# s10m/GPU-Tiled-QR-Decomposition

Hardware: AMD Instinct MI355X
Metric: fp64 QR GFLOP/s and %MFMA-peak, dense m×n, at 1/2/4/8 MI355X (higher is better)
Workload: dtype f64; 1 GPU; tiled QR 16384x16384 f64 storage, tile 256 (BASELINE configs[2]); m=16384, n=16384, tile=256, parallelism=single GPU, inputs=one resident copy per timed step, staged before the timed region, chain_segment_length=8

## Files before the change

gpu-tiled-qr-decomposition_amd/csrc/chain_asm.hpp:

```cpp
#pragma once
#ifdef TQR_C64_INC
#include TQR_C64_INC
#else
#include "chain_asm_gen.inc"
#endif

namespace tqr {

__device__ __forceinline__ __amdgpu_buffer_rsrc_t null_rsrc(const void* p) {
  const unsigned long long u = (unsigned long long)p;
  const unsigned lo = __builtin_amdgcn_readfirstlane((unsigned)u);
  const unsigned hi = __builtin_amdgcn_readfirstlane((unsigned)(u >> 32));
  return __builtin_amdgcn_make_buffer_rsrc((void*)(((unsigned long long)hi << 32) | lo), 0, 0, 0x00020000);
}

template <int B>
__device__ __forceinline__ void ca_load_strip_head(__amdgpu_buffer_rsrc_t xin, __amdgpu_buffer_rsrc_t hrs, unsigned loff) {
  if constexpr (B == 256)
    asm volatile("s_nop 4\n\t" TQR_CHAIN_ASM_STRIP_LOAD_B256 "\n\t" TQR_CHAIN_ASM_HEAD_LOAD
                 :: [loff] "v"(loff), [xin] "s"(xin), [hrs] "s"(hrs) : "memory", TQR_CHAIN_ASM_CLOBBERS);
  else
    asm volatile("s_nop 4\n\t" TQR_CHAIN_ASM_STRIP_LOAD_B128 "\n\t" TQR_CHAIN_ASM_HEAD_LOAD
                 :: [loff] "v"(loff), [xin] "s"(xin), [hrs] "s"(hrs) : "memory", TQR_CHAIN_ASM_CLOBBERS);
}

__device__ __forceinline__ unsigned sreg(unsigned v) {
  unsigned r;
  asm volatile("s_nop 1\n\tv_readfirstlane_b32 %0, %1" : "=s"(r) : "v"(v));
  return r;
}

#if TQR_CHAIN_ASM_COAL
#define TQR_CA_COAL_INS , [bpa] "v"(o.bpa), [loffc] "v"(o.loffc), [hoff] "s"(o.hoff)
#define TQR_CA_COAL_CLOB "vcc",
#else
#define TQR_CA_COAL_INS
#define TQR_CA_COAL_CLOB
#endif
struct CaGroup {
  unsigned vz, vx, vt, vl16, loff;
  const double* svsrc;
  const double* stsrc;
  unsigned sdst;
  int sw;
  __amdgpu_buffer_rsrc_t hrs;
  int goff, hsc;
  __amdgpu_buffer_rsrc_t xout, xin, hnx;
  unsigned bpa = 0, loffc = 0;
  int hoff = 0;
};
__device__ __forceinline__ unsigned coal_bpa(int lane) { return 4u * (unsigned)(((lane & 3) << 4) | (lane >> 3)); }
__device__ __forceinline__ unsigned coal_off(int lane, size_t ldm) {
  return (unsigned)(((size_t)(lane >> 3) * ldm + 2 * (lane & 7)) * sizeof(double));
}

template <int B, int KIND, int G = 0>
__device__ __forceinline__ void ca_group(const CaGroup& o) {
  unsigned m0s, st;
#define TQR_CA_INS                                                                                     \
  [vz] "v"(o.vz), [vx] "v"(o.vx), [vt] "v"(o.vt), [vl16] "v"(o.vl16), [loff] "v"(o.loff), [svsrc] "s"(o.svsrc), \
      [stsrc] "s"(o.stsrc), [sdst] "s"(o.sdst), [sw] "s"(o.sw), [hrs] "s"(o.hrs),                            \
      [goff] "s"(o.goff), [hsc] "s"(o.hsc), [xout] "s"(o.xout), [xin] "s"(o.xin),       \
      [hnx] "s"(o.hnx) TQR_CA_COAL_INS
#define TQR_CA_STMT(TEXT) \
  asm volatile(TEXT : [m0s] "=&s"(m0s), [st] "=&s"(st) : TQR_CA_INS : "memory", "scc", TQR_CA_COAL_CLOB TQR_CHAIN_ASM_CLOBBERS)
  if constexpr (KIND == 4) {
    static_assert(G >= 1 && G + 1 < B / 32, "UNMQR body: groups 1 .. NG-2");
    if constexpr (B == 256) {
      if constexpr (G == 1) TQR_CA_STMT(TQR_CHAIN_ASM_U1_B256);
      else if constexpr (G == 2) TQR_CA_STMT(TQR_CHAIN_ASM_U2_B256);
      else if constexpr (G == 3) TQR_CA_STMT(TQR_CHAIN_ASM_U3_B256);
      else if constexpr (G == 4) TQR_CA_STMT(TQR_CHAIN_ASM_U4_B256);
      else if constexpr (G == 5) TQR_CA_STMT(TQR_CHAIN_ASM_U5_B256);
      else TQR_CA_STMT(TQR_CHAIN_ASM_U6_B256);
    } else {
      if constexpr (G == 1) TQR_CA_STMT(TQR_CHAIN_ASM_U1_B128);
      else TQR_CA_STMT(TQR_CHAIN_ASM_U2_B128);
    }
  } else if constexpr (KIND == 5 || KIND == 6) {
    if constexpr (B == 256) {
      if constexpr (KIND == 5) TQR_CA_STMT(TQR_CHAIN_ASM_UHANDOVER_B256);
      else TQR_CA_STMT(TQR_CHAIN_ASM_UHANDOVERL_B256);
    } else {
      if constexpr (KIND == 5) TQR_CA_STMT(TQR_CHAIN_ASM_UHANDOVER_B128);
      else TQR_CA_STMT(TQR_CHAIN_ASM_UHANDOVERL_B128);
    }
  } else if constexpr (B == 256) {
    if constexpr (KIND == 0) TQR_CA_STMT(TQR_CHAIN_ASM_PLAIN_B256);
    else if constexpr (KIND == 1) TQR_CA_STMT(TQR_CHAIN_ASM_HANDOVER_B256);
    else if constexpr (KIND == 2) TQR_CA_STMT(TQR_CHAIN_ASM_HANDOVERL_B256);
    else TQR_CA_STMT(TQR_CHAIN_ASM_XIN_B256);
  } else {
    if constexpr (KIND == 0) TQR_CA_STMT(TQR_CHAIN_ASM_PLAIN_B128);
    else if constexpr (KIND == 1) TQR_CA_STMT(TQR_CHAIN_ASM_HANDOVER_B128);
    else if constexpr (KIND == 2) TQR_CA_STMT(TQR_CHAIN_ASM_HANDOVERL_B128);
    else TQR_CA_STMT(TQR_CHAIN_ASM_XIN_B128);
  }
#undef TQR_CA_STMT
#undef TQR_CA_INS
}

template <int B>
__device__ __forceinline__ void ca_ugroup(int g, const CaGroup& o) {
  if constexpr (B == 256) {
    switch (g) {
      case 1: ca_group<B, 4, 1>(o); break;
      case 2: ca_group<B, 4, 2>(o); break;
      case 3: ca_group<B, 4, 3>(o); break;
      case 4: ca_group<B, 4, 4>(o); break;
      case 5: ca_group<B, 4, 5>(o); break;
      default: ca_group<B, 4, 6>(o); break;
    }
  } else {
    if (g == 1) ca_group<B, 4, 1>(o);
// ... 155 lines not shown
  int* const tcs = sflag + 58;
  int* const fls = sflag + 59;
  int* const acs = sflag + 60;
  if (pw) {
    pv.reset();
    *lds_int(tcs) = -1;
    *lds_int(fls) = -1;
  }
  const bool remote = a.dist && tile_owner(k, a.world, a.cyclic) != a.rank;
  int* const rf = uni(a.Rf + (size_t)k * P * NG);
  const int ep = uni(a.epoch);
  int fl_pf = -1;
  auto ready = [&](int i_, int g_) -> bool {
    if (!remote) return pv.ensure(rc, g_, i_ - k + 1, err);
    const int fi = i_ * NG + g_;
    if (fi == fl_pf && lds_u(fls) >= ep) return true;
    return spin_ge_u(rf + fi, ep, err, true);
  };
  const unsigned lds0 = __builtin_amdgcn_readfirstlane((unsigned)(size_t)(const __attribute__((address_space(3))) void*)lds);
  const unsigned oz = (unsigned)((x * VP + y * NRI) * 8), ox = (unsigned)((y * VP + x * NRI) * 8);
  const unsigned ot = (unsigned)(G::VIMG * 8 + (x * 4 + y) * NRI * 8);
  const unsigned loff = head_off_pair<B>(ldm, 0);
  const unsigned vl16 = 16u * lane;
#if TQR_CHAIN_ASM_COAL
  const unsigned bpa = coal_bpa(lane), loffc = coal_off(lane, ldm);
  const int hoff = uni((int)(8 * ldm * sizeof(double)));
#endif
  FST(6);
  if (k == 0 && a.Uc) {
    const bool ok = pw ? spin_ge_u(&a.Uc[j], a.nxc, err) : true;
    if (!ca_sync<0, 5>(ok, pw, sflag, par)) return;
  }
  const int ifirst = seg == 0 ? k : i0;
  bool xin = false;
  bool xu = false;
  for (int i = ifirst; i < i1 || i == k; i = (i == k ? i0 : i + 1)) {
    const bool ts = i != k;
    S* const Xt = ts ? Aj + (size_t)i * B : At;
    const __amdgpu_buffer_rsrc_t hrs = head_rsrc(At + colo, ts);
    if (!xin) {
      bool ok = true;
      if (pw) {
        if (i == ifirst && seg > 0) ok = spin_ge_u(&acg[0], seg, err);
        FST(9);
        if (ok && k > 0) ok = spin_ge_u(tc(i), k, err);
        FST(8);
        if (ok) ok = ready(i, 0);
      }
      FST(j == k + 1 ? 18 : 19);
      CA_MARK(5);
      if (!ca_sync<0, 5>(ok, pw, sflag, par)) return;
      CA_RESTART();
#ifdef TQR_FLOW_STAMPS
      if (t == 0 && i == ifirst) {
        const int idx = sflag[-1];
        if (idx < (1 << 18)) g_ttl[3 * idx + 2] += (__builtin_amdgcn_s_memrealtime() - g_ttl[3 * idx]) << 16;
      }
#endif
      FST(7);
      ca_dma<B>(vimg(i, 0), timg(i, 0), sreg(lds0 + (unsigned)(buf * BUF * 8)), w, vl16);
      ca_load_strip_head<B>(uniform_rsrc(Xt + colo), hrs, loff);
      FST(4);
    }
    const int inext = uni((i == k) ? i0 : i + 1);
    const bool has_next = uni(inext < i1 ? 1 : 0) != 0;
    bool okall = true;
    for (int g = 0; g < NG && okall; ++g) {
      bool ok = true;
      CA_MARK(7);
      const bool pp = pw;
      if (pp) {
        if (g + 1 == NG && has_next && k > 0 && lds_u(tcs) < k) ok = spin_ge_u(tc(inext), k, err);
        if (ok && i == ifirst && seg > 0 && g + 1 < NG && !(g > 0 && lds_u(acs) >= seg))
          ok = spin_ge_u(&acg[g + 1], seg, err);
        if (ok) {
          if (g + 1 < NG) ok = ready(i, g + 1);
          else if (has_next) ok = ready(inext, 0);
        }
      }
      FST(j == k + 1 ? 20 : 0);
      CA_MARK(2);
      constexpr int NHO = 2 * NP + 8 < 63 ? 2 * NP + 8 : 63;
      constexpr int XL = B == 256 ? TQR_CHAIN_ASM_XLEAD_B256 : TQR_CHAIN_ASM_XLEAD_B128;
      constexpr int NHL = NP + XL + 8 < 63 ? NP + XL + 8 : 63;
// ... 20 lines not shown
        const int tg = next_test_group<NG>(g);
        const bool here = g + 2 < NG;
        if (here || has_next) {
          if (!remote) {
            if (pfw) lds_prefetch_u(rc + tg, pv.rv + tg, false);
          } else if (pw) {
            fl_pf = (here ? i : inext) * NG + tg;
            lds_prefetch_u(rf + fl_pf, fls, true);
          }
        }
        if (pw && g + 2 == NG && has_next && k > 0) lds_prefetch_u(tc(inext), tcs, false);
        if (pw && i == ifirst && seg > 0 && g + 2 < NG) lds_prefetch_u(&acg[g + 2], acs, false);
      }
      FST(7);
      CA_RESTART();
      const int gd = g + 1 < NG ? g + 1 : has_next ? 0 : g, id = g + 1 < NG ? i : has_next ? inext : i;
      const unsigned vb = lds0 + (unsigned)(buf * BUF * 8);
      CaGroup o;
      o.vz = vb + oz;
      o.vx = vb + ox;
      o.vt = vb + ot;
      o.vl16 = vl16;
      o.loff = loff;
      o.svsrc = vimg(id, gd);
      o.stsrc = timg(id, gd);
      o.sdst = sreg(lds0 + (unsigned)((buf ^ 1) * BUF * 8));
      o.sw = w;
      o.hrs = hrs;
      o.hsc = (int)sreg(has_next ? 0u : 1u);
      o.goff = uni(g * IB * 8);
#if TQR_CHAIN_ASM_COAL
      o.bpa = bpa;
      o.loffc = loffc;
      o.hoff = hoff;
#endif
      CA_MARK(3);
      const bool ue = !ts && uskip;
      if (g + 1 < NG) {
        if (ue && g > 0) {
          o.xout = uniform_rsrc(Xt + colo);
          ca_ugroup<B>(g, o);
        } else if (g == 0 && xin && late) {
          o.xin = uniform_rsrc(Xt + colo);
          ca_group<B, 3>(o);
        } else {
          ca_group<B, 0>(o);
// ... 38 lines not shown
```

gpu-tiled-qr-decomposition_amd/csrc/flow_list.hpp:

```cpp
#pragma once

#if defined(__HIPCC__)
#define TQR_HD __host__ __device__
#else
#define TQR_HD
#endif

namespace tqr {

struct Item {
  int ts, l, m, k;
};

inline bool valid_b(int b) { return b == 16 || b == 32 || b == 64 || b == 128 || b == 256; }

constexpr int T_CHAIN = 4;
constexpr int T_UP = 5, T_DOWN = 6;

template <int NW_, int IB_, int WPC_>
struct FlowShape {
  static constexpr int NW = NW_, NT = 64 * NW_, SW = 16 * NW_, IB = IB_, WPC = WPC_;
};
using ShapeW8 = FlowShape<8, 32, 1>;
using ShapeW4 = FlowShape<4, 16, 2>;
// ... 6 lines not shown

TQR_HD inline int tile_owner(int j, int world, int cyclic = 0) {
  const int blk = j / world, r = j - blk * world;
  if (cyclic) return r;
  return (blk & 1) ? world - 1 - r : r;
}

TQR_HD inline int seglen_of_chain(int k, int j, int kmax, int seglen, int seglen_la, int la_tail,
                                  int tail = 0, int tail_sl = 1) {
  if (k >= kmax - tail) return tail_sl;
  if (j != k + 1) return seglen;
  return k >= kmax - la_tail ? 1 : seglen_la;
}
TQR_HD inline bool unmqr_alone(int k, int j, int kmax, int ualone) { return j == k + 1 && k >= kmax - ualone; }
TQR_HD inline int nseg_of_chain(int k, int j, int p, int kmax, int sl, int ualone) {
  const int rows = p - k - 1;
  if (rows <= 0) return 1;
  return (rows + sl - 1) / sl + (unmqr_alone(k, j, kmax, ualone) ? 1 : 0);
}
TQR_HD inline int seg_of_row(int k, int j, int i, int kmax, int sl, int ualone) {
  return (i - k - 1) / sl + (unmqr_alone(k, j, kmax, ualone) ? 1 : 0);
}

}
```

gpu-tiled-qr-decomposition_amd/csrc/flowplan.cpp:

```cpp
#include "flowplan.hpp"

#include <cstdlib>
#include <cstring>
#include <functional>
#include <map>
#include <queue>
#include <string>
#include <tuple>
#include <unordered_map>

#include "gridscheduler.h"

namespace tqr {

int flow_shape(int dtype, int b) {
  if (dtype != TQR_F64) return 8;
  const char* e = getenv("TQR_FLOW_SHAPE");
  if (e && strcmp(e, "w4") == 0) return 4;
  if (e && strcmp(e, "r") == 0 && b == 256) return 5;
  return 8;
}

namespace {
using u64 = unsigned long long;
// ... 534 lines not shown
int tqr_flow_plan_check(int M, int N, int b, int seglen, int* ntasks, int* est_order) {
  return list_check(spec64(M, N, b, seglen), ntasks, est_order);
}

int tqr_flow_xfer_plan_check(int M, int N, int b, int seglen, int nxc, double tcol, int* ntasks, int* est_order) {
  if (nxc < 1) return TQR_EINVAL;
  return list_check(spec64(M, N, b, seglen, 1, -1, nxc, tcol), ntasks, est_order);
}

int tqr_dist_plan_check(int M, int N, int b, int seglen, int rank, int world, int* ntasks, int* nfwd) {
  if (rank < 0 || seglen < 1) return TQR_EINVAL;
  FlowPlan fp;
  if (flow_list(spec64(M, N, b, seglen, world, rank), fp) != TQR_OK) return TQR_EINVAL;
  if (ntasks) *ntasks = (int)fp.items.size();
  if (nfwd) {
    int c = 0;
    if (world > 1)
      for (auto& it : fp.items) c += (it.ts & 0xff) != T_CHAIN;
    *nfwd = c;
  }
  return TQR_OK;
}

int tqr_flow_strip_width(void) { return shape_info(flow_shape(TQR_F64, 256)).sw; }

int tqr_flow_order_check(int M, int N, int b, const int* items, int n) {
  if (M <= 0 || N <= 0 || !valid_b(b) || !items || n <= 0) return TQR_EINVAL;
  std::vector<Item> L(n);
  for (int x = 0; x < n; ++x) L[x] = Item{items[4 * x], items[4 * x + 1], items[4 * x + 2], items[4 * x + 3]};
  return flow_list_topological(L, M, N, shape_ns(flow_shape(TQR_F64, b), b)) ? 1 : 0;
}

}
```

gpu-tiled-qr-decomposition_amd/csrc/plans.hip:

```cpp
#include <hip/hip_runtime.h>

#include <algorithm>
#include <cstdio>
#include <cstdlib>
#include <cstring>
#include <mutex>
#include <new>
#include <tuple>
#include <vector>

#include "gridscheduler.h"
#include "plan.hpp"
#include "solve.hpp"
#include "tqr.h"
#include "wave_dev.hpp"

using namespace tqr;

tqr::PlanShape tqr::plan_shape(const tqr_plan* pl) { return PlanShape{pl->m, pl->n, pl->b, pl->dtype, pl->kmax, pl->capped}; }

extern "C" {

const char* tqr_strerror(int s) {
  switch (s) {
// ... 117 lines not shown
  pl->ldsU = lds_update(b);
  if (hipEventCreate(&pl->ev0) != hipSuccess || hipEventCreate(&pl->ev1) != hipSuccess ||
      hipEventCreateWithFlags(&pl->evDone, hipEventDisableTiming) != hipSuccess) {
    tqr_plan_destroy(pl); return TQR_EHIP;
  }
  pl->shape = flow_shape(dtype, b);
  pl->nt = shape_info(pl->shape).nt;
  pl->ns = shape_ns(pl->shape, b);
  pl->ng = b / shape_ib(pl->shape, b);
  if (pl->engine == TQR_ENGINE_FLOW) {
    int dev = 0;
    hipDeviceProp_t pr;
    if (hipGetDevice(&dev) != hipSuccess || hipGetDeviceProperties(&pr, dev) != hipSuccess) {
      tqr_plan_destroy(pl); return TQR_EHIP;
    }
    const int full_grid = pr.multiProcessorCount * shape_info(pl->shape).wpc;
    pl->grid = full_grid;
    if (const char* gs = getenv("TQR_FLOW_GRID")) pl->grid = std::max(1, atoi(gs));
    FlowPlan fp;
    pl->knobs = flow_knobs(pl->p, pl->q, dtype, world, pl->grid >= full_grid, 0, steps, b);
    if (const char* eca = getenv("TQR_CHAIN_ASM")) pl->chain_asm = atoi(eca) & 3;
    if (const char* eu = getenv("TQR_UNMQR_SKIP"); eu && atoi(eu) == 0 && pl->chain_asm) pl->chain_asm |= 4;
    if (const char* e32 = getenv("TQR_CHAIN32_ASM"); e32 && atoi(e32) == 0) pl->chain_asm |= 8;
    build_flow_plan(pl->p, pl->q, pl->ns, pl->ng, pl->knobs, fp, nullptr, steps);
    pl->nflow_global = (int)fp.items.size();
    pl->list_hash = flow_list_hash(fp.items);
    if (world > 1) partition_flow_plan(fp, rank, world);
    pl->nflow = (int)fp.items.size();
    pl->est_order = fp.est_order;
    pl->sync_ints = 4 + 3 * (size_t)pl->kmax * pl->ng + (size_t)pl->p * pl->q * pl->ns +
                    (size_t)pl->kmax * pl->q * pl->ns * pl->ng + (size_t)pl->q;
    if (pl->nflow <= 0 || hipMalloc(&pl->d_flow, sizeof(Item) * pl->nflow) != hipSuccess ||
        hipMalloc(&pl->d_sync, sizeof(int) * pl->sync_ints) != hipSuccess ||
        hipMalloc(&pl->d_wk, sizeof(double*) * pl->kmax) != hipSuccess) {
      tqr_plan_destroy(pl); return TQR_ENOMEM;
    }
    const bool wk_uc = world > 1 && !(getenv("TQR_DIST_WK_CACHED") && atoi(getenv("TQR_DIST_WK_CACHED")) == 1);
    for (int k = 0; k < pl->kmax; ++k) {
      double* w = nullptr;
      const size_t wb = wk_bytes(b, pl->p - k, dtype, shape_ib(pl->shape, b));
      if ((wk_uc ? hipExtMallocWithFlags((void**)&w, wb, hipDeviceMallocUncached) : hipMalloc(&w, wb)) != hipSuccess) {
        tqr_plan_destroy(pl); return TQR_ENOMEM;
      }
      pl->wk.push_back(w);
    }
    if (hipMemcpy(pl->d_wk, pl->wk.data(), sizeof(double*) * pl->kmax, hipMemcpyHostToDevice) != hipSuccess) {
// ... 103 lines not shown
```

gpu-tiled-qr-decomposition_amd/gen/gen_chain_asm.py:

```python
#!/usr/bin/env python3
import os
import sys

NW = 8
IB = 32
NRI = IB // 4
VP = IB + 2
VPB = VP * 8

sys.path.insert(0, os.path.dirname(os.path.abspath(__file__)))
import gfx950_hazards as HZ

W_MF_C, W_MF_AB, W_MF_VALU, W_MF_ST = HZ.F64["srcc"], HZ.F64["srcab"], HZ.F64["valu"], HZ.F64["vmem"]
W_VALU_MF, W_VALU_ST, W_ST_WAR, W_M0 = HZ.VALU_TO_MFMA, HZ.VALU_TO_STORE, HZ.STORE_WAR, HZ.M0_TO_LDS_DMA

OP0, Z0, WR0, H0, X0 = 32, 80, 96, 112, 128
HP0 = 128
VTMP1, VDMA, VTMP2 = 96, 97, 80
VLO = 32


AG = 512


# ... 121 lines not shown

    def wait_lgkm(self, tags):
        idx = [self.lgkm.index(t) for t in tags if t in self.lgkm]
        if not idx:
            return
        k = len(self.lgkm) - 1 - max(idx)
        assert k <= 15
        self.emit(f"s_waitcnt lgkmcnt({k})")
        self.lgkm = self.lgkm[len(self.lgkm) - k:] if k else []

    def text(self):
        return "\\n\\t".join(self.lines)


class Body:

    def __init__(self, B, handover, nw=NW, xbank=None, resident=False, after_switch=False, xlead=None, xin_from=None,
                 skip=0, early_st=(), early_ld=()):
        self.B, self.NKS, self.NP = B, B // 4, B // 8
        self.handover = handover
        self.nw = nw
        self.X0 = X0 if xbank is None else AG + 128 * xbank
        self.coal = COAL and nw == 8 and xbank is None
        self.s = Stream()
        vimg = (B * VP + 127) // 128 * 128
        self.VIMG = vimg
        self.NIV, self.NIT = vimg // 128, (16 * NRI * NRI + 127) // 128
        self.PV, self.PT = -(-self.NIV // nw), -(-self.NIT // nw)
        self.STEPS = self.PV + self.PT
        self.s.vm = [f"X{p}" for p in range(self.NP)] + ["H"]
        self.xlead, self.xin_from = xlead, xin_from
        if xin_from is not None:
            self.s.vm = [f"X{p}" for p in range(xin_from)] + ["H"]
        self.skip, self.early_st, self.early_ld = skip, list(early_st), list(early_ld)
        assert skip % 8 == 0 and 0 <= skip < self.NKS and (xin_from is None or not skip)
        self.resident = resident
        if resident:
            assert not handover and xbank is not None and nw == 4
            self.s.vm = [f"X{p}" for p in RES_LD_SCHED[-1]] if after_switch else []

    def p1_slot(self, ks):
        return OP0 + 16 * (ks % 3)

    def t_slot(self, kb):
        return OP0 + 16 * (1 + kb % 2)

# ... 60 lines not shown

        K0 = self.skip
        dma_at = {}
        for m in range(self.STEPS):
            dma_at.setdefault(K0 + int((m + 0.5) * (NKS - K0) / self.STEPS), []).append(m)
        vtmp_set = False

        def need_vtmp(ks):
            nonlocal vtmp_set
            if ks < NKS and ks * 4 * VPB + 48 >= 65536 and not vtmp_set:
                s.emit(f"v_add_u32 v{VTMP1}, 0x8000, %[vz]")
                vtmp_set = True

        early = [("st", p) for p in self.early_st] + [("ld", p) for p in self.early_ld]
        for ks in range(K0, min(K0 + D, NKS)):
            need_vtmp(ks)
            p1_reads(ks)
        for ks in range(K0, NKS):
            nxt = ks + D
            need_vtmp(nxt)
            if self.xin_from is not None and ks % 2 == 0:
                for p in range(self.xin_from, self.NP):
                    if max(0, 2 * (p - self.xin_from)) == ks:
                        s.vmem_load(self.X0 + 4 * p, f"buffer_load_dwordx4 {vq(self.X0 + 4 * p)}, %[loff], %[xin], 0 "
                                    f"offen offset:{64 * p} sc1 nt", f"XI{p}")
            if ks % 2 == 0:
                s.wait_vm(f"X{ks // 2}")
            s.wait_lgkm([f"z{ks}.{h}" for h in range(4)])
            sl = self.p1_slot(ks)
            for r in range(NRI):
                s.mfma(Z0 + 2 * r, sl + 2 * r, self.X0 + 2 * ks, "0" if ks == K0 else Z0 + 2 * r)
                if nxt < NKS and r in (1, 3, 5, 7):
                    h = (r - 1) // 2
                    off = nxt * 4 * VPB + 16 * h
                    base, o = self.lds("%[vz]", off, VTMP1)
                    s.ds_read(self.p1_slot(nxt) + 4 * h, base, o, f"z{nxt}.{h}")
                if r == 2:
                    for m in dma_at.get(ks, []):
                        self.dma_step(m)
                if r == 5 and early:
                    for _ in range(-(-len(early) // (NKS - ks))):
                        self.strip_io(*early.pop(0))
        assert not early
        def t_reads(kb):
            for h in range(4):
                s.ds_read(self.t_slot(kb) + 4 * h, "%[vt]", kb * 1024 + 16 * h, f"t{kb}.{h}")

        units = [(b, half, pp) for b in range(K0 // 4, NKS // 4) for half in range(2) for pp in range(2)]
# ... 143 lines not shown
            self.s.emit("s_waitcnt lgkmcnt(0)")

    CT = (H0, H0 + 8)

    def coal_bperm(self, q):
        s = self.s
        for h in range(2):
            t = self.CT[h]
            for d in range(4):
                s.ds_bperm(t + d, self.X0 + 4 * (2 * q) + d, 32 * h, f"bp{q}.{h}.a{d}")
                s.ds_bperm(t + 4 + d, self.X0 + 4 * (2 * q + 1) + d, 32 * h, f"bp{q}.{h}.b{d}")

    def coal_store(self, q):
        s = self.s
        for h in range(2):
            t = self.CT[h]
            s.wait_lgkm([f"bp{q}.{h}.{ab}{d}" for ab in "ab" for d in range(4)])
            for d in range(4):
                s.valu_cnd(t + d, t + d, t + 4 + d)
            so = "%[hoff]" if h else "0"
            s.vmem_store(t, f"buffer_store_dwordx4 {vq(t)}, %[loffc], %[xout], {so} offen offset:{128 * q} sc1",
                         f"XS{2 * q + h}")

    def strip_io(self, kind, p):
        s = self.s
        r = self.X0 + 4 * p
        if kind == "st":
            s.vmem_store(r, f"buffer_store_dwordx4 {vq(r)}, %[loff], %[xout], 0 offen offset:{64 * p} sc1", f"XS{p}")
        else:
            s.vmem_load(r, f"buffer_load_dwordx4 {vq(r)}, %[loff], %[xin], 0 offen offset:{64 * p} sc1 nt", f"XL{p}")


def simulate(B, bodies, nelem=3, seglen_last=True, ubodies=None):
    NG, NP = B // IB, B // 8
    plain, ho = bodies[0], bodies[1]
    xin = bodies[2] if len(bodies) > 2 else None
    lead = ho.xlead if ho.xlead is not None else NP
    out = []
    stored, loaded = {}, {}

    def wait(k):
        while len(out) > k:
            out.pop(0)

    def done(pred, what):
        bad = [o for o in out if pred(o)]
        assert not bad, f"B={B}: {what}: {bad[:3]} still outstanding"

    def play(body, e, g):
        for ev in body.s.events:
            if ev[0] == "vm":
                tag = ev[1]
                if tag.startswith("D"):
# ... 47 lines not shown
            else:
                play(ho if g + 1 == NG else xin if (xin is not None and g == 0 and e > 0) else plain, e, g)
    wait(0)
    for e in range(nelem):
        assert sorted(stored.get(e, [])) == list(range(NP)), f"B={B}: strip stores of element {e}"
        if e > 0:
            assert sorted(loaded.get(e, [])) == list(range(NP)), f"B={B}: strip loads of element {e}"
    return True


def dma_job(B, nw=NW):
    body = Body(B, False, nw)
    st = body.s
    st.emit("s_nop 4")
    st.emit("s_mov_b32 %[m0s], m0")
    for m in range(body.STEPS):
        body.dma_step(m)
    st.emit("s_mov_b32 m0, %[m0s]")
    return st.text()


def strip_load(B, x0=X0):
    NP = B // 8
    lines = [f"buffer_load_dwordx4 {vq(x0 + 4 * p)}, %[loff], %[xin], 0 offen offset:{64 * p} sc1 nt" for p in range(NP)]
    return "\\n\\t".join(lines)


def head_load():
    lines = [f"buffer_load_dwordx4 {vq(H0 + 4 * h)}, %[loff], %[hrs], 0 offen offset:{64 * h} sc1" for h in range(4)]
    return "\\n\\t".join(lines)


def strip_store(B, x0=X0):
    NP = B // 8
    lines = [f"buffer_store_dwordx4 {vq(x0 + 4 * p)}, %[loff], %[xout], 0 offen offset:{64 * p} sc1" for p in range(NP)]
    lines.append("s_nop 1")
    return "\\n\\t".join(lines)


STAMPS = bool(os.environ.get("GEN_STAMPS"))
COAL = bool(os.environ.get("GEN_COALESCE"))
XLEAD = int(os.environ.get("GEN_XLEAD", "2"))
NOPRIO = bool(os.environ.get("GEN_NOPRIO"))
PWPRIO = bool(os.environ.get("GEN_PWPRIO"))
PRIOREV = bool(os.environ.get("GEN_PRIOREV"))

RES_ST_SCHED = [list(range(0, 16)), list(range(16, 32))]
RES_LD_SCHED = [list(range(0, 6)), list(range(6, 12)), list(range(12, 17)), list(range(17, 22)),
                list(range(22, 27)), list(range(27, 32))]


def _lines(ls):
    return "\\n\\t".join(ls)


def res_xst(g, bank):
    x0 = 128 * bank
    ls = ["s_nop 4"]
    ls += [f"buffer_store_dwordx4 a[{x0 + 4 * p}:{x0 + 4 * p + 3}], %[loff], %[xout], 0 offen offset:{64 * p} sc1"
           for p in RES_ST_SCHED[g]]
    return _lines(ls)

# ... 6 lines not shown
    return _lines(ls)


def res_head(g, store):
    ls = ["s_nop 4"]
    for h in range(4):
        r = HP0 + 16 * g + 4 * h
        op = "buffer_store_dwordx4" if store else "buffer_load_dwordx4"
        ls.append(f"{op} v[{r}:{r + 3}], %[loff], %[hrs], 0 offen offset:{256 * g + 64 * h} sc1")
    if store:
        ls.append("s_nop 1")
    return _lines(ls)


def res_park_zero():
    return _lines([f"v_mov_b64 v[{r}:{r + 1}], 0" for r in range(HP0, 256, 2)])


def res_park_from(bank):
    return _lines(["s_nop 7"] + [f"v_accvgpr_read_b32 v{HP0 + i}, a{128 * bank + i}" for i in range(128)] + ["s_nop 1"])


def main():
    out = sys.argv[1] if len(sys.argv) > 1 else "csrc/chain_asm_gen.inc"
    parts = ["// GENERATED by gen/gen_chain_asm.py -- do not edit. fp64 chain group bodies (gfx950).", "#pragma once"]
    stats = []
    for B in (128, 256):
        built = {}
        for ho in (False, True):
            body = Body(B, ho)
            s = body.build()
            built[ho] = body
            name = f"TQR_CHAIN_ASM_{'HANDOVER' if ho else 'PLAIN'}_B{B}"
            parts.append(f'#define {name} "{s.text()}"')
            nm = sum(1 for l in s.lines if l.startswith("v_mfma"))
            nn = sum(int(l.split()[1]) + 1 for l in s.lines if l.startswith("s_nop"))
            stats.append(f"// {name}: {len(s.lines)} lines, {nm} MFMAs, {nn} nop states, {s.clock} issue slots")
        for n in (1, 2, 3, 5):
            simulate(B, (built[False], built[True]), nelem=n)
        lead = XLEAD
        hol = Body(B, True, xlead=lead)
        hol.build()
        xb = Body(B, False, xin_from=lead)
        xb.build()
        for n in (1, 2, 3, 5):
            simulate(B, (built[False], hol, xb), nelem=n)
        for nm, bd in ((f"TQR_CHAIN_ASM_HANDOVERL_B{B}", hol), (f"TQR_CHAIN_ASM_XIN_B{B}", xb)):
            parts.append(f'#define {nm} "{bd.s.text()}"')
            nmf = sum(1 for l in bd.s.lines if l.startswith("v_mfma"))
            stats.append(f"// {nm}: {len(bd.s.lines)} lines, {nmf} MFMAs, {bd.s.clock} issue slots")
        NG = B // IB
        for late in (False, True):
            ub = {}
            for g in range(1, NG):
                lo = 4 * g
                if g + 1 < NG:
                    ub[g] = Body(B, False, skip=8 * g, early_st=range(4 * (g - 1), lo))
                else:
                    ub[g] = Body(B, True, xlead=lead if late else None, skip=8 * g, early_st=range(4 * (g - 1), lo),
                                 early_ld=[p for p in range(lo) if not late or p < lead])
                ub[g].build()
            for n in (1, 2, 3, 5):
                if late:
                    simulate(B, (built[False], hol, xb), nelem=n, ubodies=ub)
                else:
                    simulate(B, (built[False], built[True]), nelem=n, ubodies=ub)
            names = [(f"TQR_CHAIN_ASM_UHANDOVER{'L' if late else ''}_B{B}", ub[NG - 1])]
            parts.append(f"#define TQR_CHAIN_ASM_UHANDOVER{'L' if late else ''}_SYNC_B{B} {ub[NG - 1].sync_after()}")
            if not late:
                names += [(f"TQR_CHAIN_ASM_U{g}_B{B}", ub[g]) for g in range(1, NG - 1)]
            for nm, bd in names:
                parts.append(f'#define {nm} "{bd.s.text()}"')
                nmf = sum(1 for l in bd.s.lines if l.startswith("v_mfma"))
                stats.append(f"// {nm}: {len(bd.s.lines)} lines, {nmf} MFMAs, {bd.s.clock} issue slots")
        parts.append(f"#define TQR_CHAIN_ASM_XLEAD_B{B} {lead}")
        if B == 128:
            parts.append(f"#define TQR_CHAIN_ASM_COAL {1 if COAL else 0}")
        parts.append(f'#define TQR_CHAIN_ASM_DMA_B{B} "{dma_job(B)}"')
        parts.append(f'#define TQR_CHAIN_ASM_STRIP_LOAD_B{B} "{strip_load(B)}"')
        parts.append(f'#define TQR_CHAIN_ASM_STRIP_STORE_B{B} "{strip_store(B)}"')
    parts.append(f'#define TQR_CHAIN_ASM_HEAD_LOAD "{head_load()}"')
    regs = ", ".join(f'"v{i}"' for i in range(VLO, 256))
    parts.append(f"#define TQR_CHAIN_ASM_CLOBBERS {regs}")
    B = 256
    built = {}
    for ho in (False, True):
        body = Body(B, ho, nw=4, xbank=0)
        s = body.build()
        built[ho] = body
        name = f"TQR_CHAIN_ASM4_{'HANDOVER' if ho else 'PLAIN'}_B{B}"
        parts.append(f'#define {name} "{s.text()}"')
        nm = sum(1 for l in s.lines if l.startswith("v_mfma"))
        nn = sum(int(l.split()[1]) + 1 for l in s.lines if l.startswith("s_nop"))
        stats.append(f"// {name}: {len(s.lines)} lines, {nm} MFMAs, {nn} nop states, {s.clock} issue slots")
    for n in (1, 2, 3, 5):
        simulate(B, (built[False], built[True]), nelem=n)
    parts.append(f'#define TQR_CHAIN_ASM4_DMA_B{B} "{dma_job(B, 4)}"')
    parts.append(f'#define TQR_CHAIN_ASM4_STRIP_LOAD_B{B} "{strip_load(B, AG)}"')
    regs4 = ", ".join([f'"v{i}"' for i in range(VLO, 128)] + [f'"a{i}"' for i in range(256)])
    parts.append(f"#define TQR_CHAIN_ASM4_CLOBBERS {regs4}")
    for bank in (0, 1):
        for sw in (False, True):
            body = Body(B, False, nw=4, xbank=bank, resident=True, after_switch=sw)
# ... 31 lines not shown
```

gpu-tiled-qr-decomposition_amd/tqr.py:

```python
import ctypes
import os

import numpy as np

HERE = os.path.dirname(os.path.abspath(__file__))
LIB_PATH = os.path.join(HERE, os.environ.get("TQR_LIB", "libtqr.so"))

TQR_F32, TQR_F64 = 0, 1
QRS, SAPP, QRD, DAPP = 0, 1, 2, 3
TASK_AVAIL, TASK_NONE, TASK_DONE = 0, 1, 2
READY, DOING, DONE, NONE, NOTASKS = 0, 1, 2, 3, 4

_lib = None
_P = ctypes.c_void_p
_I = ctypes.c_int


class TQRError(RuntimeError):
    pass


class Task(ctypes.Structure):
    _fields_ = [("taskType", _I), ("l", _I), ("m", _I), ("k", _I), ("taskStatus", _I)]

# ... 16 lines not shown
    except Exception:
        pass
    if not os.path.exists(LIB_PATH):
        raise TQRError(f"{LIB_PATH} is missing — build it with __graft_entry__.build() "
                       "(make -C gpu-tiled-qr-decomposition_amd)")
    L = ctypes.CDLL(LIB_PATH)
    L.tqr_strerror.restype = ctypes.c_char_p
    L.tqr_version.restype = ctypes.c_char_p
    L.tqr_total_tasks.restype = ctypes.c_long
    L.tqr_sched_total_tasks.restype = ctypes.c_long
    L.initScheduler.restype = ctypes.POINTER(Task)
    L.tqr_plan_create.argtypes = [ctypes.POINTER(_P), _I, _I, _I, _I]
    L.tqr_plan_create_steps.argtypes = [ctypes.POINTER(_P), _I, _I, _I, _I, _I]
    L.tqr_plan_create_steps.restype = _I
    L.tqr_plan_create_engine.argtypes = [ctypes.POINTER(_P), _I, _I, _I, _I, _I]
    L.tqr_plan_create_engine.restype = _I
    L.tqr_plan_info.argtypes = [_P, ctypes.POINTER(_I), ctypes.POINTER(_I), ctypes.POINTER(_I), ctypes.POINTER(_I)]
    L.tqr_plan_info.restype = _I
    L.tqr_plan_set_tasks.argtypes = [_P, _P, _I]
    L.tqr_plan_set_tasks.restype = _I
    if hasattr(L, "tqr_plan_get_tasks"):
        L.tqr_plan_get_tasks.argtypes = [_P, _P, _I]
        L.tqr_plan_get_tasks.restype = _I
    L.tqr_plan_debug_workspace.argtypes = [_P, _I, _P, ctypes.c_size_t]
    L.tqr_plan_debug_workspace.restype = _I
    L.cudaQRFull.argtypes = [_P, _I, _I]
    L.cudaQRFull.restype = None
    L.tqr_plan_steps.argtypes = [_P]
    L.tqr_plan_steps.restype = _I
    L.tqr_plan_execute.argtypes = [_P, _P, _I, _P, _P]
    L.tqr_plan_destroy.argtypes = [_P]
    L.tqr_plan_set_profile.argtypes = [_P, _I]
    L.tqr_plan_stats.argtypes = [_P, ctypes.POINTER(_I), ctypes.POINTER(ctypes.c_double),
                                 ctypes.POINTER(_I), ctypes.POINTER(ctypes.c_double)]
    L.tqr_fill_randzo.argtypes = [_I, _P, _I, _I, _I, ctypes.c_ulonglong, _P]
    L.tqr_fill_randzo_cols.argtypes = [_I, _P, _I, _I, _I, ctypes.c_ulonglong, ctypes.c_long, _P]
    L.tqr_dist_local_cols.argtypes = [_P]
    for nm in ("tqr_tile_geqrt", "tqr_tile_unmqr", "tqr_tile_tsqrt", "tqr_tile_tsmqr"):
        getattr(L, nm).restype = _I
    L.tqr_dist_plan_create.argtypes = [ctypes.POINTER(_P), _I, _I, _I, _I, _I, _I]
    L.tqr_dist_handle_bytes.argtypes = [_P]
    L.tqr_dist_handle_bytes.restype = ctypes.c_size_t
    L.tqr_dist_export.argtypes = [_P, ctypes.c_char_p, ctypes.c_size_t]
    L.tqr_dist_import.argtypes = [_P, ctypes.c_char_p, ctypes.c_size_t]
    L.tqr_dist_reset.argtypes = [_P, _P]
    L.tqr_dist_probe.argtypes = [_P, _I, ctypes.POINTER(ctypes.c_ulonglong)]
# ... 333 lines not shown

class FlowListSpec(ctypes.Structure):
    _fields_ = [(f, _I) for f in ("M", "N", "b", "dtype", "seglen", "world", "rank", "full", "nxc")] + \
               [("tcol", ctypes.c_double)]


def flow_list(M, N, b, dtype=TQR_F64, seglen=0, world=1, rank=-1, full=1, nxc=0, tcol=0.0, steps=0):
    spec = FlowListSpec(M, N, b, dtype, seglen, world, rank, full, nxc, tcol)
    if steps:
        def export(items, cap):
            return lib().tqr_flow_list_export_steps(ctypes.byref(spec), steps, items, cap)
    else:
        def export(items, cap):
            return lib().tqr_flow_list_export(ctypes.byref(spec), items, cap)
    n = export(None, 0)
    if n < 0:
        check(n, "tqr_flow_list_export")
    items = np.zeros((n, 4), dtype=np.int32)
    if export(_ptr(items), n) != n:
        raise TQRError("tqr_flow_list_export: the list changed between two calls")
    return items


def plan_info(plan):
    v = [_I() for _ in range(4)]
    check(lib().tqr_plan_info(plan.h, *[ctypes.byref(x) for x in v]), "tqr_plan_info")
    return dict(zip(("engine", "ntasks", "est_order", "grid"), (x.value for x in v)))


def plan_tasks(plan):
    n = lib().tqr_plan_get_tasks(plan.h, None, 0)
    if n < 0:
        check(n, "tqr_plan_get_tasks")
    items = np.zeros((n, 4), dtype=np.int32)
    if lib().tqr_plan_get_tasks(plan.h, _ptr(items), n) != n:
        raise TQRError("tqr_plan_get_tasks: the list changed between two calls")
    return items


def fill_randzo(A, m, n, seed, ldda=None, stream=None, col0=0):
    check(lib().tqr_fill_randzo_cols(_dtype_code(A.dtype), _ptr(A), m, n, ldda or m, seed, col0, _P(stream or 0)),
          "tqr_fill_randzo_cols")


def geqrt_host(A, b, with_tau=True, m=None, tau=None, engine=None):
    n, ldm = A.shape
# ... 482 lines not shown
```

include/tqr.h:

```cpp
#ifndef TQR_H
#define TQR_H
#include <stddef.h>
#ifdef __cplusplus
extern "C" {
#endif

enum tqr_status {
    TQR_OK = 0,
    TQR_EINVAL = -1,
    TQR_ENOMEM = -2,
    TQR_EHIP = -3,
    TQR_ENODEV = -4,
    TQR_ERCCL = -5
};
enum tqr_dtype { TQR_F32 = 0, TQR_F64 = 1 };

const char* tqr_strerror(int status);
const char* tqr_version(void);

typedef struct tqr_plan tqr_plan;

int tqr_plan_create(tqr_plan** plan, int m, int n, int b, int dtype);
enum tqr_engine { TQR_ENGINE_DEFAULT = -1, TQR_ENGINE_WAVES = 0, TQR_ENGINE_FLOW = 1 };
int tqr_plan_create_engine(tqr_plan** plan, int m, int n, int b, int dtype, int engine);
int tqr_plan_create_steps(tqr_plan** plan, int m, int n, int b, int dtype, int steps);
int tqr_plan_steps(const tqr_plan* plan);
void tqr_plan_destroy(tqr_plan* plan);

int tqr_plan_execute(tqr_plan* plan, void* dA, int ldda, void* dtau_compact, void* stream);

int tqr_plan_status(tqr_plan* plan, void* stream);
int tqr_plan_info(const tqr_plan* plan, int* engine, int* ntasks, int* est_order, int* grid);

int tqr_flow_plan_check(int M, int N, int b, int seglen, int* ntasks, int* est_order);
int tqr_flow_strip_width(void);
int tqr_flow_plan_export(int M, int N, int b, int seglen, int* items, int cap);
typedef struct tqr_flow_list_spec {
    int M, N, b, dtype, seglen, world, rank, full, nxc;
    double tcol;
} tqr_flow_list_spec;
int tqr_flow_list_export(const tqr_flow_list_spec* spec, int* items, int cap);
int tqr_flow_list_export_steps(const tqr_flow_list_spec* spec, int steps, int* items, int cap);
int tqr_plan_set_tasks(tqr_plan* plan, const int* items, int n);
int tqr_plan_get_tasks(tqr_plan* plan, int* items, int cap);
int tqr_flow_order_check(int M, int N, int b, const int* items, int n);
int tqr_plan_debug_workspace(const tqr_plan* plan, int k, void* host, size_t bytes);

int tqr_plan_set_profile(tqr_plan* plan, int on);
int tqr_plan_stats(const tqr_plan* plan, int* nlaunch_update, double* ms_update, int* nlaunch_panel,
                   double* ms_panel);

long tqr_total_tasks(int m, int n, int b);

typedef struct tqr_apply tqr_apply;
enum tqr_trans { TQR_NOTRANS = 0, TQR_TRANS = 1 };
int tqr_apply_create(tqr_apply** ap, int m, int n, int b, int dtype);
size_t tqr_apply_workspace_bytes(const tqr_apply* ap);
int tqr_apply_prepare(tqr_apply* ap, const void* dA, int ldda, const void* dtau_compact, void* stream);
int tqr_apply_q(tqr_apply* ap, int trans, const void* dA, int ldda, void* dC, int nrhs, int lddc, void* stream);
// ... 95 lines not shown
```

Baseline: 51530 GFLOP/s.

## Permute strip load/store lane addressing so each lane covers whole cache lines

Adds an alternate strip memory layout for fp64 B=256 chain kernels. Lanes are remapped so that each group of lanes touches contiguous 128-byte lines, with an odd-pair scalar offset. Strips written in one step are stored in the permuted layout and read back the same way in later steps. The layout is enabled by default when chain_asm mode 2 and shape 8 are in use. The goal is better memory coalescing for strip I/O, at the cost of added address registers and layout-tracking logic that must stay consistent between producer and consumer tiles.

```diff
diff --git a/gpu-tiled-qr-decomposition_amd/csrc/chain_asm.hpp b/gpu-tiled-qr-decomposition_amd/csrc/chain_asm.hpp
--- a/gpu-tiled-qr-decomposition_amd/csrc/chain_asm.hpp
+++ b/gpu-tiled-qr-decomposition_amd/csrc/chain_asm.hpp
@@ -4,6 +4,7 @@
 #else
 #include "chain_asm_gen.inc"
 #endif
+#include "chain_asm_lines_gen.inc"
 
 namespace tqr {
 
@@ -14,20 +15,26 @@
   return __builtin_amdgcn_make_buffer_rsrc((void*)(((unsigned long long)hi << 32) | lo), 0, 0, 0x00020000);
 }
 
-template <int B>
-__device__ __forceinline__ void ca_load_strip_head(__amdgpu_buffer_rsrc_t xin, __amdgpu_buffer_rsrc_t hrs, unsigned loff) {
-  if constexpr (B == 256)
-    asm volatile("s_nop 4\n\t" TQR_CHAIN_ASM_STRIP_LOAD_B256 "\n\t" TQR_CHAIN_ASM_HEAD_LOAD
-                 :: [loff] "v"(loff), [xin] "s"(xin), [hrs] "s"(hrs) : "memory", TQR_CHAIN_ASM_CLOBBERS);
-  else
-    asm volatile("s_nop 4\n\t" TQR_CHAIN_ASM_STRIP_LOAD_B128 "\n\t" TQR_CHAIN_ASM_HEAD_LOAD
-                 :: [loff] "v"(loff), [xin] "s"(xin), [hrs] "s"(hrs) : "memory", TQR_CHAIN_ASM_CLOBBERS);
-}
-
 __device__ __forceinline__ unsigned sreg(unsigned v) {
   unsigned r;
   asm volatile("s_nop 1\n\tv_readfirstlane_b32 %0, %1" : "=s"(r) : "v"(v));
   return r;
+}
+
+template <int B>
+__device__ __forceinline__ void ca_load_strip_head(__amdgpu_buffer_rsrc_t xin, __amdgpu_buffer_rsrc_t hrs, unsigned loff,
+                                                   unsigned va1, unsigned xs) {
+  if constexpr (B == 256)
+    asm volatile("s_nop 4\n\t" TQR_CHAIN_ASML_STRIP_LOAD_B256 "\n\t" TQR_CHAIN_ASM_HEAD_LOAD
+                 :: [loff] "v"(loff), [va1] "v"(va1), [xs] "s"(xs), [xin] "s"(xin), [hrs] "s"(hrs)
+                 : "memory", TQR_CHAIN_ASM_CLOBBERS);
+  else
+    asm volatile("s_nop 4\n\t" TQR_CHAIN_ASM_STRIP_LOAD_B128 "\n\t" TQR_CHAIN_ASM_HEAD_LOAD
+                 :: [loff] "v"(loff), [xin] "s"(xin), [hrs] "s"(hrs) : "memory", TQR_CHAIN_ASM_CLOBBERS);
+}
+template <int B>
+__device__ __forceinline__ void ca_load_strip_head(__amdgpu_buffer_rsrc_t xin, __amdgpu_buffer_rsrc_t hrs, unsigned loff) {
+  ca_load_strip_head<B>(xin, hrs, loff, loff, sreg(0u));
 }
 
 #if TQR_CHAIN_ASM_COAL
@@ -39,6 +46,11 @@
 #endif
 struct CaGroup {
   unsigned vz, vx, vt, vl16, loff;
+  unsigned va0, va1, xso, xs;
+  __device__ __forceinline__ void standard_strips() {
+    va0 = va1 = loff;
+    xso = xs = sreg(0u);
+  }
   const double* svsrc;
   const double* stsrc;
   unsigned sdst;
@@ -59,6 +71,7 @@
   unsigned m0s, st;
 #define TQR_CA_INS                                                                                     \
   [vz] "v"(o.vz), [vx] "v"(o.vx), [vt] "v"(o.vt), [vl16] "v"(o.vl16), [loff] "v"(o.loff), [svsrc] "s"(o.svsrc), \
+      [va0] "v"(o.va0), [va1] "v"(o.va1), [xso] "s"(o.xso), [xs] "s"(o.xs),                                  \
       [stsrc] "s"(o.stsrc), [sdst] "s"(o.sdst), [sw] "s"(o.sw), [hrs] "s"(o.hrs),                            \
       [goff] "s"(o.goff), [hsc] "s"(o.hsc), [xout] "s"(o.xout), [xin] "s"(o.xin),       \
       [hnx] "s"(o.hnx) TQR_CA_COAL_INS
@@ -67,29 +80,29 @@
   if constexpr (KIND == 4) {
     static_assert(G >= 1 && G + 1 < B / 32, "UNMQR body: groups 1 .. NG-2");
     if constexpr (B == 256) {
-      if constexpr (G == 1) TQR_CA_STMT(TQR_CHAIN_ASM_U1_B256);
-      else if constexpr (G == 2) TQR_CA_STMT(TQR_CHAIN_ASM_U2_B256);
-      else if constexpr (G == 3) TQR_CA_STMT(TQR_CHAIN_ASM_U3_B256);
-      else if constexpr (G == 4) TQR_CA_STMT(TQR_CHAIN_ASM_U4_B256);
-      else if constexpr (G == 5) TQR_CA_STMT(TQR_CHAIN_ASM_U5_B256);
-      else TQR_CA_STMT(TQR_CHAIN_ASM_U6_B256);
+      if constexpr (G == 1) TQR_CA_STMT(TQR_CHAIN_ASML_U1_B256);
+      else if constexpr (G == 2) TQR_CA_STMT(TQR_CHAIN_ASML_U2_B256);
+      else if constexpr (G == 3) TQR_CA_STMT(TQR_CHAIN_ASML_U3_B256);
+      else if constexpr (G == 4) TQR_CA_STMT(TQR_CHAIN_ASML_U4_B256);
+      else if constexpr (G == 5) TQR_CA_STMT(TQR_CHAIN_ASML_U5_B256);
+      else TQR_CA_STMT(TQR_CHAIN_ASML_U6_B256);
     } else {
       if constexpr (G == 1) TQR_CA_STMT(TQR_CHAIN_ASM_U1_B128);
       else TQR_CA_STMT(TQR_CHAIN_ASM_U2_B128);
     }
   } else if constexpr (KIND == 5 || KIND == 6) {
     if constexpr (B == 256) {
-      if constexpr (KIND == 5) TQR_CA_STMT(TQR_CHAIN_ASM_UHANDOVER_B256);
-      else TQR_CA_STMT(TQR_CHAIN_ASM_UHANDOVERL_B256);
+      if constexpr (KIND == 5) TQR_CA_STMT(TQR_CHAIN_ASML_UHANDOVER_B256);
+      else TQR_CA_STMT(TQR_CHAIN_ASML_UHANDOVERL_B256);
     } else {
       if constexpr (KIND == 5) TQR_CA_STMT(TQR_CHAIN_ASM_UHANDOVER_B128);
       else TQR_CA_STMT(TQR_CHAIN_ASM_UHANDOVERL_B128);
     }
   } else if constexpr (B == 256) {
     if constexpr (KIND == 0) TQR_CA_STMT(TQR_CHAIN_ASM_PLAIN_B256);
-    else if constexpr (KIND == 1) TQR_CA_STMT(TQR_CHAIN_ASM_HANDOVER_B256);
-    else if constexpr (KIND == 2) TQR_CA_STMT(TQR_CHAIN_ASM_HANDOVERL_B256);
-    else TQR_CA_STMT(TQR_CHAIN_ASM_XIN_B256);
+    else if constexpr (KIND == 1) TQR_CA_STMT(TQR_CHAIN_ASML_HANDOVER_B256);
+    else if constexpr (KIND == 2) TQR_CA_STMT(TQR_CHAIN_ASML_HANDOVERL_B256);
+    else TQR_CA_STMT(TQR_CHAIN_ASML_XIN_B256);
   } else {
     if constexpr (KIND == 0) TQR_CA_STMT(TQR_CHAIN_ASM_PLAIN_B128);
     else if constexpr (KIND == 1) TQR_CA_STMT(TQR_CHAIN_ASM_HANDOVER_B128);
@@ -291,6 +304,12 @@
   const unsigned ot = (unsigned)(G::VIMG * 8 + (x * 4 + y) * NRI * 8);
   const unsigned loff = head_off_pair<B>(ldm, 0);
   const unsigned vl16 = 16u * lane;
+  const bool lines = B == 256 && (uni(a.chain_asm) & 16) != 0;
+  const int kmx = uni(a.kmax);
+  const unsigned lperm = strip_lane_off(1, lane, ldm * sizeof(S));
+  const unsigned dperm = strip_odd_off(1, ldm * sizeof(S));
+  const bool ldp = lines && k >= 1;
+  const unsigned va1 = ldp ? lperm : loff, xs = ldp ? dperm : 0u;
 #if TQR_CHAIN_ASM_COAL
   const unsigned bpa = coal_bpa(lane), loffc = coal_off(lane, ldm);
   const int hoff = uni((int)(8 * ldm * sizeof(double)));
@@ -328,7 +347,7 @@
 #endif
       FST(7);
       ca_dma<B>(vimg(i, 0), timg(i, 0), sreg(lds0 + (unsigned)(buf * BUF * 8)), w, vl16);
-      ca_load_strip_head<B>(uniform_rsrc(Xt + colo), hrs, loff);
+      ca_load_strip_head<B>(uniform_rsrc(Xt + colo), hrs, loff, ts ? va1 : loff, sreg(ts ? xs : 0u));
       FST(4);
     }
     const int inext = uni((i == k) ? i0 : i + 1);
@@ -395,6 +414,11 @@
       o.vt = vb + ot;
       o.vl16 = vl16;
       o.loff = loff;
+      const bool stp = lines && strip_permuted(i, j, k, kmx);
+      o.va0 = stp ? lperm : loff;
+      o.xso = sreg(stp ? dperm : 0u);
+      o.va1 = va1;
+      o.xs = sreg(xs);
       o.svsrc = vimg(id, gd);
       o.stsrc = timg(id, gd);
       o.sdst = sreg(lds0 + (unsigned)((buf ^ 1) * BUF * 8));
diff --git a/gpu-tiled-qr-decomposition_amd/csrc/flow_list.hpp b/gpu-tiled-qr-decomposition_amd/csrc/flow_list.hpp
--- a/gpu-tiled-qr-decomposition_amd/csrc/flow_list.hpp
+++ b/gpu-tiled-qr-decomposition_amd/csrc/flow_list.hpp
@@ -52,4 +52,11 @@
   return (i - k - 1) / sl + (unmqr_alone(k, j, kmax, ualone) ? 1 : 0);
 }
 
+TQR_HD inline bool strip_permuted(int i, int j, int k, int kmax) { return i > k + 1 && j > k + 1 && k + 1 < kmax; }
+TQR_HD inline unsigned strip_lane_off(int layout, int lane, size_t col) {
+  const unsigned x = (unsigned)lane >> 4, c = (unsigned)lane & 15;
+  return layout ? (unsigned)((2 * x + (c >> 3)) * col + 16 * (c & 7)) : (unsigned)(c * col + 16 * x);
 }
+TQR_HD inline unsigned strip_odd_off(int layout, size_t col) { return layout ? (unsigned)(8 * col - 64) : 0u; }
+
+}
diff --git a/gpu-tiled-qr-decomposition_amd/csrc/flowplan.cpp b/gpu-tiled-qr-decomposition_amd/csrc/flowplan.cpp
--- a/gpu-tiled-qr-decomposition_amd/csrc/flowplan.cpp
+++ b/gpu-tiled-qr-decomposition_amd/csrc/flowplan.cpp
@@ -580,6 +580,21 @@
   return TQR_OK;
 }
 
+int tqr_flow_strip_layout(int p, int q, int steps, int i, int j, int k) {
+  if (p < 1 || q < 1 || steps < 0 || steps > std::min(p, q)) return TQR_EINVAL;
+  const int kmax = flow_kmax(p, q, steps);
+  if (k < 0 || k >= kmax || i < k || i >= p || j <= k || j >= q) return TQR_EINVAL;
+  return strip_permuted(i, j, k, kmax) ? 1 : 0;
+}
+
+long tqr_flow_strip_offset(int layout, int pair, int lane, long ld) {
+  if ((layout != 0 && layout != 1) || pair < 0 || pair >= 32 || lane < 0 || lane >= 64 || ld < 256 ||
+      (size_t)ld * 8 * 16 >= ((size_t)1 << 31))
+    return TQR_EINVAL;
+  const size_t col = (size_t)ld * 8;
+  return (long)(strip_lane_off(layout, lane, col) + ((pair & 1) ? strip_odd_off(layout, col) : 0u) + 64u * (unsigned)pair);
+}
+
 int tqr_flow_strip_width(void) { return shape_info(flow_shape(TQR_F64, 256)).sw; }
 
 int tqr_flow_order_check(int M, int N, int b, const int* items, int n) {
diff --git a/gpu-tiled-qr-decomposition_amd/csrc/plans.hip b/gpu-tiled-qr-decomposition_amd/csrc/plans.hip
--- a/gpu-tiled-qr-decomposition_amd/csrc/plans.hip
+++ b/gpu-tiled-qr-decomposition_amd/csrc/plans.hip
@@ -163,6 +163,10 @@
     if (const char* eca = getenv("TQR_CHAIN_ASM")) pl->chain_asm = atoi(eca) & 3;
     if (const char* eu = getenv("TQR_UNMQR_SKIP"); eu && atoi(eu) == 0 && pl->chain_asm) pl->chain_asm |= 4;
     if (const char* e32 = getenv("TQR_CHAIN32_ASM"); e32 && atoi(e32) == 0) pl->chain_asm |= 8;
+    if (dtype == TQR_F64 && b == 256 && pl->shape == 8 && (pl->chain_asm & 3) == 2) {
+      const char* el = getenv("TQR_STRIP_LINES");
+      if (!el || atoi(el) != 0) pl->chain_asm |= 16;
+    }
     build_flow_plan(pl->p, pl->q, pl->ns, pl->ng, pl->knobs, fp, nullptr, steps);
     pl->nflow_global = (int)fp.items.size();
     pl->list_hash = flow_list_hash(fp.items);
diff --git a/gpu-tiled-qr-decomposition_amd/gen/gen_chain_asm.py b/gpu-tiled-qr-decomposition_amd/gen/gen_chain_asm.py
--- a/gpu-tiled-qr-decomposition_amd/gen/gen_chain_asm.py
+++ b/gpu-tiled-qr-decomposition_amd/gen/gen_chain_asm.py
@@ -167,6 +167,7 @@
         self.nw = nw
         self.X0 = X0 if xbank is None else AG + 128 * xbank
         self.coal = COAL and nw == 8 and xbank is None
+        self.own_addr = LINES and nw == 8 and xbank is None
         self.s = Stream()
         vimg = (B * VP + 127) // 128 * 128
         self.VIMG = vimg
@@ -273,8 +274,8 @@
             if self.xin_from is not None and ks % 2 == 0:
                 for p in range(self.xin_from, self.NP):
                     if max(0, 2 * (p - self.xin_from)) == ks:
-                        s.vmem_load(self.X0 + 4 * p, f"buffer_load_dwordx4 {vq(self.X0 + 4 * p)}, %[loff], %[xin], 0 "
-                                    f"offen offset:{64 * p} sc1 nt", f"XI{p}")
+                        s.vmem_load(self.X0 + 4 * p, f"buffer_load_dwordx4 {vq(self.X0 + 4 * p)}, "
+                                    f"{self.xaddr('ld', p, '%[xin]')} sc1 nt", f"XI{p}")
             if ks % 2 == 0:
                 s.wait_vm(f"X{ks // 2}")
             s.wait_lgkm([f"z{ks}.{h}" for h in range(4)])
@@ -464,13 +465,30 @@
             s.vmem_store(t, f"buffer_store_dwordx4 {vq(t)}, %[loffc], %[xout], {so} offen offset:{128 * q} sc1",
                          f"XS{2 * q + h}")
 
+    def xaddr(self, kind, p, rsrc):
+        return xaddr_text(kind if self.own_addr else None, p, rsrc)
+
     def strip_io(self, kind, p):
         s = self.s
         r = self.X0 + 4 * p
         if kind == "st":
-            s.vmem_store(r, f"buffer_store_dwordx4 {vq(r)}, %[loff], %[xout], 0 offen offset:{64 * p} sc1", f"XS{p}")
+            s.vmem_store(r, f"buffer_store_dwordx4 {vq(r)}, {self.xaddr('st', p, '%[xout]')} sc1", f"XS{p}")
         else:
-            s.vmem_load(r, f"buffer_load_dwordx4 {vq(r)}, %[loff], %[xin], 0 offen offset:{64 * p} sc1 nt", f"XL{p}")
+            s.vmem_load(r, f"buffer_load_dwordx4 {vq(r)}, {self.xaddr('ld', p, '%[xin]')} sc1 nt", f"XL{p}")
+
+
+def xaddr_text(kind, p, rsrc):
+    if kind is None:
+        return f"%[loff], {rsrc}, 0 offen offset:{64 * p}"
+    vo, so = ("%[va0]", "%[xso]") if kind == "st" else ("%[va1]", "%[xs]")
+    return f"{vo}, {rsrc}, {so if p & 1 else 0} offen offset:{64 * p}"
+
+
+def strip_lines_map(p, lane, col):
+    x, c = lane >> 4, lane & 15
+    lane_off = (2 * x + (c >> 3)) * col + 16 * (c & 7)
+    odd = 8 * col - 64
+    return lane_off + (odd if p & 1 else 0) + 64 * p
 
 
 def simulate(B, bodies, nelem=3, seglen_last=True, ubodies=None):
@@ -564,7 +582,8 @@
 
 def strip_load(B, x0=X0):
     NP = B // 8
-    lines = [f"buffer_load_dwordx4 {vq(x0 + 4 * p)}, %[loff], %[xin], 0 offen offset:{64 * p} sc1 nt" for p in range(NP)]
+    kind = "ld" if LINES and x0 == X0 else None
+    lines = [f"buffer_load_dwordx4 {vq(x0 + 4 * p)}, {xaddr_text(kind, p, '%[xin]')} sc1 nt" for p in range(NP)]
     return "\\n\\t".join(lines)
 
 
@@ -580,6 +599,7 @@
     return "\\n\\t".join(lines)
 
 
+LINES = False
 STAMPS = bool(os.environ.get("GEN_STAMPS"))
 COAL = bool(os.environ.get("GEN_COALESCE"))
 XLEAD = int(os.environ.get("GEN_XLEAD", "2"))
@@ -632,16 +652,27 @@
 
 
 def main():
-    out = sys.argv[1] if len(sys.argv) > 1 else "csrc/chain_asm_gen.inc"
+    global LINES
+    args = sys.argv[1:]
+    LINES = bool(args) and args[0] == "--lines"
+    if LINES:
+        args = args[1:]
+    out = args[0] if args else ("csrc/chain_asm_lines_gen.inc" if LINES else "csrc/chain_asm_gen.inc")
     parts = ["// GENERATED by gen/gen_chain_asm.py -- do not edit. fp64 chain group bodies (gfx950).", "#pragma once"]
+    if LINES:
+        parts[0] = ("// GENERATED by gen/gen_chain_asm.py --lines -- do not edit. fp64 chain group bodies (gfx950, "
+                    "8 waves, B = 256) with strip address operands.")
+    PRE = "TQR_CHAIN_ASML" if LINES else "TQR_CHAIN_ASM"
     stats = []
-    for B in (128, 256):
+    for B in ((256,) if LINES else (128, 256)):
         built = {}
         for ho in (False, True):
             body = Body(B, ho)
             s = body.build()
             built[ho] = body
-            name = f"TQR_CHAIN_ASM_{'HANDOVER' if ho else 'PLAIN'}_B{B}"
+            name = f"{PRE}_{'HANDOVER' if ho else 'PLAIN'}_B{B}"
+            if LINES and not ho:
+                continue
             parts.append(f'#define {name} "{s.text()}"')
             nm = sum(1 for l in s.lines if l.startswith("v_mfma"))
             nn = sum(int(l.split()[1]) + 1 for l in s.lines if l.startswith("s_nop"))
@@ -655,7 +686,7 @@
         xb.build()
         for n in (1, 2, 3, 5):
             simulate(B, (built[False], hol, xb), nelem=n)
-        for nm, bd in ((f"TQR_CHAIN_ASM_HANDOVERL_B{B}", hol), (f"TQR_CHAIN_ASM_XIN_B{B}", xb)):
+        for nm, bd in ((f"{PRE}_HANDOVERL_B{B}", hol), (f"{PRE}_XIN_B{B}", xb)):
             parts.append(f'#define {nm} "{bd.s.text()}"')
             nmf = sum(1 for l in bd.s.lines if l.startswith("v_mfma"))
             stats.append(f"// {nm}: {len(bd.s.lines)} lines, {nmf} MFMAs, {bd.s.clock} issue slots")
@@ -675,20 +706,30 @@
                     simulate(B, (built[False], hol, xb), nelem=n, ubodies=ub)
                 else:
                     simulate(B, (built[False], built[True]), nelem=n, ubodies=ub)
-            names = [(f"TQR_CHAIN_ASM_UHANDOVER{'L' if late else ''}_B{B}", ub[NG - 1])]
-            parts.append(f"#define TQR_CHAIN_ASM_UHANDOVER{'L' if late else ''}_SYNC_B{B} {ub[NG - 1].sync_after()}")
+            names = [(f"{PRE}_UHANDOVER{'L' if late else ''}_B{B}", ub[NG - 1])]
+            if not LINES:
+                parts.append(f"#define TQR_CHAIN_ASM_UHANDOVER{'L' if late else ''}_SYNC_B{B} {ub[NG - 1].sync_after()}")
             if not late:
-                names += [(f"TQR_CHAIN_ASM_U{g}_B{B}", ub[g]) for g in range(1, NG - 1)]
+                names += [(f"{PRE}_U{g}_B{B}", ub[g]) for g in range(1, NG - 1)]
             for nm, bd in names:
                 parts.append(f'#define {nm} "{bd.s.text()}"')
                 nmf = sum(1 for l in bd.s.lines if l.startswith("v_mfma"))
                 stats.append(f"// {nm}: {len(bd.s.lines)} lines, {nmf} MFMAs, {bd.s.clock} issue slots")
+        if LINES:
+            parts.append(f'#define {PRE}_STRIP_LOAD_B{B} "{strip_load(B)}"')
+            continue
         parts.append(f"#define TQR_CHAIN_ASM_XLEAD_B{B} {lead}")
         if B == 128:
             parts.append(f"#define TQR_CHAIN_ASM_COAL {1 if COAL else 0}")
         parts.append(f'#define TQR_CHAIN_ASM_DMA_B{B} "{dma_job(B)}"')
         parts.append(f'#define TQR_CHAIN_ASM_STRIP_LOAD_B{B} "{strip_load(B)}"')
         parts.append(f'#define TQR_CHAIN_ASM_STRIP_STORE_B{B} "{strip_store(B)}"')
+    if LINES:
+        parts[2:2] = stats
+        with open(out, "w") as f:
+            f.write("\n".join(parts) + "\n")
+        print("\n".join(stats))
+        return
     parts.append(f'#define TQR_CHAIN_ASM_HEAD_LOAD "{head_load()}"')
     regs = ", ".join(f'"v{i}"' for i in range(VLO, 256))
     parts.append(f"#define TQR_CHAIN_ASM_CLOBBERS {regs}")
diff --git a/gpu-tiled-qr-decomposition_amd/tqr.py b/gpu-tiled-qr-decomposition_amd/tqr.py
--- a/gpu-tiled-qr-decomposition_amd/tqr.py
+++ b/gpu-tiled-qr-decomposition_amd/tqr.py
@@ -62,6 +62,11 @@
     if hasattr(L, "tqr_plan_get_tasks"):
         L.tqr_plan_get_tasks.argtypes = [_P, _P, _I]
         L.tqr_plan_get_tasks.restype = _I
+    if hasattr(L, "tqr_flow_strip_layout"):
+        L.tqr_flow_strip_layout.argtypes = [_I] * 6
+        L.tqr_flow_strip_layout.restype = _I
+        L.tqr_flow_strip_offset.argtypes = [_I, _I, _I, ctypes.c_long]
+        L.tqr_flow_strip_offset.restype = ctypes.c_long
     L.tqr_plan_debug_workspace.argtypes = [_P, _I, _P, ctypes.c_size_t]
     L.tqr_plan_debug_workspace.restype = _I
     L.cudaQRFull.argtypes = [_P, _I, _I]
@@ -441,6 +446,20 @@
     return items
 
 
+def strip_layout(p, q, steps, i, j, k):
+    r = lib().tqr_flow_strip_layout(p, q, steps, i, j, k)
+    if r < 0:
+        check(r, "tqr_flow_strip_layout")
+    return r
+
+
+def strip_offset(layout, pair, lane, ld):
+    r = lib().tqr_flow_strip_offset(layout, pair, lane, ld)
+    if r < 0:
+        check(r, "tqr_flow_strip_offset")
+    return r
+
+
 def plan_info(plan):
     v = [_I() for _ in range(4)]
     check(lib().tqr_plan_info(plan.h, *[ctypes.byref(x) for x in v]), "tqr_plan_info")
diff --git a/include/tqr.h b/include/tqr.h
--- a/include/tqr.h
+++ b/include/tqr.h
@@ -35,6 +35,8 @@
 int tqr_flow_plan_check(int M, int N, int b, int seglen, int* ntasks, int* est_order);
 int tqr_flow_strip_width(void);
 int tqr_flow_plan_export(int M, int N, int b, int seglen, int* items, int cap);
+int tqr_flow_strip_layout(int p, int q, int steps, int i, int j, int k);
+long tqr_flow_strip_offset(int layout, int pair, int lane, long ld);
 typedef struct tqr_flow_list_spec {
     int M, N, b, dtype, seglen, world, rank, full, nxc;
     double tcol;
```

Measured after the change: 52620 GFLOP/s (median of 6 runs). +2.1%, better.
